# hip-satomi/microbeSEG

Measured on AMD Instinct MI355X. Metric: training crops/sec (256px), higher is better.
Workload: dtype f32; 1 GPU; BASELINE configs[1]: DU-Net distance-map training step, filters [64, 1024], 256x256 crops, per-GPU batch 32, fp32, relu/bn, SmoothL1x2 + Adam(amsgrad); global_batch=32, parallelism=dp1, launch=eager

## Files before the change

### microbeseg_amd/csrc/igemm.hip

```cpp
#include "common.h"
#include "igemm_common.h"
#include "bf16_affine.h"

int igemm_p8_try(const MsegIgemm& p, int tr, int m_fastest, int cus, hipStream_t st);

__device__ float g_ident_scale[MSEG_MAX_CH];
__device__ float g_ident_shift[MSEG_MAX_CH];
__global__ void init_ident_kernel() {
  for (int i = blockIdx.x * blockDim.x + threadIdx.x; i < MSEG_MAX_CH; i += gridDim.x * blockDim.x) {
    g_ident_scale[i] = 1.f;
    g_ident_shift[i] = 0.f;
  }
}


template <int BM, int BN, bool PER_SAMPLE, bool GENERIC_ACT>
__global__ __launch_bounds__(256) void igemm_kernel(const MsegIgemm p) {
  using Cfg = IgemmCfg<BM, BN>;
  constexpr int STAGE = (BM + BN) * LDS_STRIDE;
  __shared__ __attribute__((aligned(16))) float lds[2 * STAGE + 4];
  unsigned* tapmask_s = reinterpret_cast<unsigned*>(lds + 2 * STAGE);

  const int tid = threadIdx.x;
  const int lane = tid & 63;
  const int wave = tid >> 6;
  const int wm = wave / Cfg::WN, wn = wave % Cfg::WN;

  const int M = p.NB * p.Ho * p.Wo;
  const int ntiles_n = (p.Ngemm + BN - 1) / BN;
  const int lid = (int)xcd_logical_id(blockIdx.x, gridDim.x);
  const int tile_m = lid / ntiles_n;
  const int tile_n = lid - tile_m * ntiles_n;
  const int m0 = tile_m * BM, n0 = tile_n * BN;

  const int T = p.KH * p.KW;
  const int srow = tid >> 3;
  const int scol = tid & 7;

  const TapGeom geom = make_geom(p);
  RowInfo rows[Cfg::AROWS];
#pragma unroll
  for (int i = 0; i < Cfg::AROWS; ++i) rows[i] = decode_row(p, m0 + srow + 32 * i, M);

  unsigned tapmask = (T >= 32) ? 0xffffffffu : ((1u << T) - 1u);
  if (p.mode == MSEG_MODE_TCONV && p.stride == 2) {
    if (tid == 0) *tapmask_s = 0u;
    __syncthreads();
    unsigned mine = 0u;
    for (int t = 0; t < T; ++t) {
      const int ky = t / p.KW, kx = t - ky * p.KW;
      bool any = false;
#pragma unroll
      for (int i = 0; i < Cfg::AROWS; ++i) {
        int iy, ix;
        any |= tap_coord(geom, rows[i], ky, kx, iy, ix);
      }
      if (any) mine |= (1u << t);
    }
    if (mine) atomicOr(tapmask_s, mine);
    __syncthreads();
    tapmask = *tapmask_s;
    __syncthreads();
  }

  f32x16 acc[Cfg::MB][Cfg::NB];
#pragma unroll
  for (int a = 0; a < Cfg::MB; ++a)
#pragma unroll
    for (int b = 0; b < Cfg::NB; ++b)
#pragma unroll
      for (int r = 0; r < 16; ++r) acc[a][b][r] = 0.f;

  const int nchunks = (p.Cin + KC - 1) / KC;
  const int C0 = p.src[0].C;

  constexpr int NSC = PER_SAMPLE ? Cfg::AROWS : 1;
  float4 ra[Cfg::AROWS], rb[Cfg::BROWS], rsc[NSC], rsh[NSC];
  unsigned amask = 0u;
  int ract = 0;

  auto issue = [&](int chunk, int t, int ky, int kx) {
    const int c = chunk * KC + scol * 4;
    const bool cvalid = c < p.Cin;
    const bool s1 = (p.nsrc > 1) & (c >= C0);
    const float* sptr = s1 ? p.src[1].ptr : p.src[0].ptr;
    const float* sscale = s1 ? p.src[1].scale : p.src[0].scale;
    const float* sshift = s1 ? p.src[1].shift : p.src[0].shift;
    const unsigned sC = (unsigned)(s1 ? p.src[1].C : p.src[0].C);
    const unsigned sss = (unsigned)(s1 ? p.src[1].ss : p.src[0].ss);
    ract = s1 ? p.src[1].act : p.src[0].act;
    const unsigned cl = cvalid ? (unsigned)(s1 ? c - C0 : c) : 0u;
    amask = 0u;
#pragma unroll
    for (int i = 0; i < Cfg::AROWS; ++i) {
      int iy, ix;
      const bool ok = cvalid & tap_coord(geom, rows[i], ky, kx, iy, ix);
      const unsigned pix = (unsigned)((rows[i].n * p.Hi + iy) * p.Wi + ix) & (0u - (unsigned)ok);
      const size_t off = (size_t)pix * sC + (cl & (0u - (unsigned)ok));
      ra[i] = *reinterpret_cast<const float4*>(sptr + off);
      amask |= (unsigned)ok << i;
    }
    const bool has_aff = sscale != nullptr;
    const float* scp = has_aff ? sscale : g_ident_scale;
    const float* shp = has_aff ? sshift : g_ident_shift;
#pragma unroll
    for (int i = 0; i < NSC; ++i) {
      const unsigned n = PER_SAMPLE ? (unsigned)(rows[i].n < 0 ? 0 : rows[i].n) : 0u;
      const size_t o = (size_t)n * (has_aff ? sss : 0u) + cl;
      rsc[i] = *reinterpret_cast<const float4*>(scp + o);
      rsh[i] = *reinterpret_cast<const float4*>(shp + o);
    }
    const float* wt = p.w + ((size_t)t * p.Npad) * p.Kpad;
#pragma unroll
    for (int i = 0; i < Cfg::BROWS; ++i)
      rb[i] = *reinterpret_cast<const float4*>(wt + (size_t)(n0 + srow + 32 * i) * p.Kpad + c);
  };

  auto commit = [&](float* As, float* Bs) {
    const float lo = (ract == MSEG_ACT_RELU) ? 0.f : -3.402823466e38f;
#pragma unroll
    for (int i = 0; i < Cfg::AROWS; ++i) {
      float4 v = ra[i];
      if (GENERIC_ACT) {
        v = act_fwd4(v, ract);
      } else {
        v.x = fmaxf(v.x, lo); v.y = fmaxf(v.y, lo); v.z = fmaxf(v.z, lo); v.w = fmaxf(v.w, lo);
      }
      const float4 sc = rsc[PER_SAMPLE ? i : 0], sh = rsh[PER_SAMPLE ? i : 0];
      const bool ok = (amask >> i) & 1u;
      v.x = ok ? v.x * sc.x + sh.x : 0.f;
      v.y = ok ? v.y * sc.y + sh.y : 0.f;
      v.z = ok ? v.z * sc.z + sh.z : 0.f;
      v.w = ok ? v.w * sc.w + sh.w : 0.f;
      *reinterpret_cast<float4*>(As + (srow + 32 * i) * LDS_STRIDE + scol * 4) = v;
    }
#pragma unroll
    for (int i = 0; i < Cfg::BROWS; ++i)
      *reinterpret_cast<float4*>(Bs + (srow + 32 * i) * LDS_STRIDE + scol * 4) = rb[i];
  };

  struct Pos { int chunk, t, ky, kx; };
  const int KWm1 = p.KW - 1;
  auto advance = [&](Pos q, bool& ok) -> Pos {
    ok = true;
    for (;;) {
      const int wrap = (q.kx == KWm1) ? 1 : 0;
      q.t += 1;
      q.kx = wrap ? 0 : q.kx + 1;
      q.ky += wrap;
      if (q.t >= T) {
        q.t = 0; q.ky = 0; q.kx = 0; q.chunk += 1;
        if (q.chunk >= nchunks) { ok = false; return q; }
      }
      if (tapmask & (1u << q.t)) return q;
    }
  };

  Pos pos = {0, -1, 0, -1};
  bool have = false;
  if (tapmask != 0u) pos = advance(pos, have);
  int cur = 0;
  if (have) {
    issue(pos.chunk, pos.t, pos.ky, pos.kx);
    commit(lds, lds + BM * LDS_STRIDE);
  }
  __syncthreads();

#ifdef MSEG_ABLATE
  const int abl = p.Cq >> 16;
  if ((abl & 16) && ((blockIdx.x >> 8) & 1)) {
    __builtin_amdgcn_s_sleep(48);
  }
  long long t_issue = 0, t_mfma = 0, t_commit = 0, t_bar = 0;
#define STAMP(var) do { if (abl & 32) { __builtin_amdgcn_sched_barrier(0); var = __builtin_amdgcn_s_memtime(); __builtin_amdgcn_s_waitcnt(0xC07F); __builtin_amdgcn_sched_barrier(0); } } while (0)
  long long s0 = 0, s1 = 0, s2 = 0, s3 = 0, s4 = 0;
#else
#define STAMP(var)
#endif
  const int li = lane & 31, lh = lane >> 5;
  while (have) {
    bool have_next;
    const Pos nxt = advance(pos, have_next);
    if (have_next) pos = nxt;
    STAMP(s0);
#ifdef MSEG_ABLATE
    if (!(abl & 1))
#endif
    issue(pos.chunk, pos.t, pos.ky, pos.kx);
    STAMP(s1);

    const float* As = lds + cur * STAGE;
    const float* Bs = As + BM * LDS_STRIDE;
#pragma unroll
    for (int kk = 0; kk < KC / 8; ++kk) {
      float4 af[Cfg::MB], bf[Cfg::NB];
#pragma unroll
      for (int a = 0; a < Cfg::MB; ++a)
        af[a] = *reinterpret_cast<const float4*>(As + (wm * Cfg::TM + a * 32 + li) * LDS_STRIDE + kk * 8 + lh * 4);
#pragma unroll
      for (int b = 0; b < Cfg::NB; ++b)
        bf[b] = *reinterpret_cast<const float4*>(Bs + (wn * Cfg::TN + b * 32 + li) * LDS_STRIDE + kk * 8 + lh * 4);
#ifdef MSEG_ABLATE
      if (abl & 4) { asm volatile("" :: "v"(af[0].x), "v"(bf[0].x)); continue; }
#endif
#pragma unroll
      for (int a = 0; a < Cfg::MB; ++a)
#pragma unroll
        for (int b = 0; b < Cfg::NB; ++b) {
          acc[a][b] = __builtin_amdgcn_mfma_f32_32x32x2f32(af[a].x, bf[b].x, acc[a][b], 0, 0, 0);
          acc[a][b] = __builtin_amdgcn_mfma_f32_32x32x2f32(af[a].y, bf[b].y, acc[a][b], 0, 0, 0);
          acc[a][b] = __builtin_amdgcn_mfma_f32_32x32x2f32(af[a].z, bf[b].z, acc[a][b], 0, 0, 0);
          acc[a][b] = __builtin_amdgcn_mfma_f32_32x32x2f32(af[a].w, bf[b].w, acc[a][b], 0, 0, 0);
        }
    }
    float* An = lds + (cur ^ 1) * STAGE;
#ifdef MSEG_ABLATE
    STAMP(s2);
    if (!(abl & 8)) commit(An, An + BM * LDS_STRIDE);
    STAMP(s3);
    if (!(abl & 2)) __syncthreads();
    STAMP(s4);
    t_issue += s1 - s0; t_mfma += s2 - s1; t_commit += s3 - s2; t_bar += s4 - s3;
#else
    commit(An, An + BM * LDS_STRIDE);
    __syncthreads();
#endif
    cur ^= 1;
    have = have_next;
  }

#ifdef MSEG_ABLATE
  if ((abl & 32) && p.dst1 && lane == 0 && blockIdx.x < 1024) {
    float* dbg = p.dst1 + ((size_t)blockIdx.x * 4 + wave) * 4;
    dbg[0] = (float)t_issue; dbg[1] = (float)t_mfma; dbg[2] = (float)t_commit; dbg[3] = (float)t_bar;
  }
#endif
  igemm_epilogue<IgemmCfg<BM, BN>>(acc, m0, n0, wm, wn, lane, M);
}

template <int BM, int BN, int TR, bool PER_SAMPLE, bool SB = false>
__global__ __launch_bounds__(256) void igemm_fast_kernel(const MsegIgemm p) {
  using Cfg = IgemmCfg<BM, BN>;
  constexpr int STAGE = (BM + BN) * LDS_STRIDE;
  __shared__ __attribute__((aligned(16))) float lds[(SB ? 1 : 2) * STAGE];

  const int tid = threadIdx.x;
  const int lane = tid & 63;
  const int wave = tid >> 6;
  const int wm = wave / Cfg::WN, wn = wave % Cfg::WN;
  const int M = p.NB * p.Ho * p.Wo;
  const int ntiles_n = (p.Ngemm + BN - 1) / BN;
  const int lid = (int)xcd_logical_id(blockIdx.x, gridDim.x);
  const int tile_m = lid / ntiles_n;
  const int tile_n = lid - tile_m * ntiles_n;
  const int m0 = tile_m * BM, n0 = tile_n * BN;
  const int T = p.KH * p.KW;
  const int srow = tid >> 3, scol = tid & 7;

  const TapGeom geom = make_geom(p);
  const long long tile_px = tile_base_pixel(p, geom, m0, M);
  int pix0[Cfg::AROWS];
  int rown[Cfg::AROWS];
  unsigned vmask[Cfg::AROWS];
#pragma unroll
  for (int i = 0; i < Cfg::AROWS; ++i) {
    const RowInfo r = decode_row(p, m0 + srow + 32 * i, M);
    const int iy0 = (r.oy * geom.sm - geom.dir * geom.pad) >> geom.sh, ix0 = (r.ox * geom.sm - geom.dir * geom.pad) >> geom.sh;
    pix0[i] = (int)(((long long)r.n * p.Hi + iy0) * p.Wi + ix0 - tile_px);
    rown[i] = r.n < 0 ? 0 : r.n;
    unsigned mk = 0u;
    for (int t = 0; t < T; ++t) {
      const int ky = t / p.KW, kx = t - ky * p.KW;
      int iy, ix;
      mk |= (unsigned)tap_coord(geom, r, ky, kx, iy, ix) << t;
    }
    vmask[i] = mk;
  }

  f32x16 acc[Cfg::MB][Cfg::NB];
#pragma unroll
  for (int a = 0; a < Cfg::MB; ++a)
#pragma unroll
    for (int b = 0; b < Cfg::NB; ++b)
#pragma unroll
      for (int r = 0; r < 16; ++r) acc[a][b][r] = 0.f;

  const int nchunks = (p.Cin + KC - 1) / KC;
  const int C0 = p.src[0].C;
  const unsigned OOB = 0x80000000u;

  const __amdgpu_buffer_rsrc_t rs0 = __builtin_amdgcn_make_buffer_rsrc(
      const_cast<float*>(p.src[0].ptr + tile_px * p.src[0].C), 0, 0x7ffffff0, 0x00020000);
  const __amdgpu_buffer_rsrc_t rs1 = __builtin_amdgcn_make_buffer_rsrc(
      const_cast<float*>((p.nsrc > 1 ? p.src[1].ptr : p.src[0].ptr) + tile_px * (p.nsrc > 1 ? p.src[1].C : p.src[0].C)), 0,
      0x7ffffff0, 0x00020000);
  const __amdgpu_buffer_rsrc_t rsw = __builtin_amdgcn_make_buffer_rsrc(const_cast<float*>(p.w), 0,
                                                                        T * p.Npad * p.Kpad * 4, 0x00020000);
  unsigned wvoff[Cfg::BROWS];
#pragma unroll
  for (int i = 0; i < Cfg::BROWS; ++i) wvoff[i] = ((unsigned)(n0 + srow + 32 * i) * (unsigned)p.Kpad + scol * 4u) * 4u;

  constexpr int NSC = (TR == 0) ? 1 : (PER_SAMPLE ? Cfg::AROWS : 1);
  float4 ra[Cfg::AROWS], rb[Cfg::BROWS], rsc[NSC], rsh[NSC];
  float rm[Cfg::AROWS];
  unsigned rowoff[Cfg::AROWS];
  int ract = 0;
  int cur_chunk = -1;
// ... 1994 lines not shown
  }
  auto tap_at = [&](int j) -> unsigned { return (unsigned)((j < 8 ? taplist >> (8 * j) : taplist_hi >> (8 * (j - 8))) & 0xffull); };
  int chunk = 0, j = 0;
  const int nsteps = nchunks * nlive;
  unsigned e0 = tap_at(0);
  issue(0, (int)(e0 & 15u), (int)((e0 >> 4) & 3u), (int)(e0 >> 6));
  commit(lds, lds + BM * HB_STRIDE);
  __syncthreads();
  int cur = 0;
  const int li = lane & 31, lh = lane >> 5;
  for (int step = 0; step < nsteps; ++step) {
    if (step + 1 < nsteps) {
      j += 1;
      if (j >= nlive) { j = 0; ++chunk; }
    }
    e0 = tap_at(j);
    issue(chunk, (int)(e0 & 15u), (int)((e0 >> 4) & 3u), (int)(e0 >> 6));

    const __bf16* As = lds + cur * STAGE;
    const __bf16* Bs = As + BM * HB_STRIDE;
#pragma unroll
    for (int kk = 0; kk < KC / 16; ++kk) {
      bf16x8 af[Cfg::MB], bf[Cfg::NB];
#pragma unroll
      for (int a = 0; a < Cfg::MB; ++a)
        af[a] = *reinterpret_cast<const bf16x8*>(As + (wm * Cfg::TM + a * 32 + li) * HB_STRIDE + kk * 16 + lh * 8);
#pragma unroll
      for (int b = 0; b < Cfg::NB; ++b)
        bf[b] = *reinterpret_cast<const bf16x8*>(Bs + (wn * Cfg::TN + b * 32 + li) * HB_STRIDE + kk * 16 + lh * 8);
#pragma unroll
      for (int a = 0; a < Cfg::MB; ++a)
#pragma unroll
        for (int b = 0; b < Cfg::NB; ++b)
          acc[a][b] = __builtin_amdgcn_mfma_f32_32x32x16_bf16(af[a], bf[b], acc[a][b], 0, 0, 0);
    }
    __bf16* An = lds + (cur ^ 1) * STAGE;
    commit(An, An + BM * HB_STRIDE);
    __syncthreads();
    cur ^= 1;
  }
  igemm_epilogue<IgemmCfg<BM, BN>>(acc, m0, n0, wm, wn, lane, M);
}

__global__ void igemm_splitk_reduce_kernel(const float* __restrict__ ws, int ksplit, size_t M, int N,
                                           const float* __restrict__ bias, float* __restrict__ dst0, int ld0, int acc0,
                                           float* __restrict__ dst1, int ld1, int acc1, int split, int d16) {
  const int N4 = N >> 2;
  const size_t total = M * (size_t)N4;
  for (size_t i = (size_t)blockIdx.x * blockDim.x + threadIdx.x; i < total; i += (size_t)gridDim.x * blockDim.x) {
    const size_t m = i / N4;
    const int n = (int)(i - m * N4) * 4;
    float4 s = *reinterpret_cast<const float4*>(ws + m * N + n);
    for (int k = 1; k < ksplit; ++k) {
      const float4 v = *reinterpret_cast<const float4*>(ws + ((size_t)k * M + m) * N + n);
      s.x += v.x; s.y += v.y; s.z += v.z; s.w += v.w;
    }
    if (bias) { s.x += bias[n]; s.y += bias[n + 1]; s.z += bias[n + 2]; s.w += bias[n + 3]; }
    const bool second = n >= split;
    void* base = second ? (void*)dst1 : (void*)dst0;
    const size_t e = second ? m * ld1 + (n - split) : m * ld0 + n;
    if (second ? acc1 : acc0) {
      const float4 o = ld_f4_rt(base, e, d16);
      s.x += o.x; s.y += o.y; s.z += o.z; s.w += o.w;
    }
    st_f4_rt(base, e, s, d16);
  }
}

static int check_src(const MsegSrc& s) {
  if (!s.ptr || s.C <= 0 || (s.C & 3)) return MSEG_EINVAL;
  if (s.dtype != MSEG_ST_F32 && s.dtype != MSEG_ST_BF16) return MSEG_EINVAL;
  if (s.dtype == MSEG_ST_BF16 && (s.C & 7)) return MSEG_EINVAL;
  if ((s.scale == nullptr) != (s.shift == nullptr)) return MSEG_EINVAL;
  if (s.scale && (s.ss & 3)) return MSEG_EINVAL;
  return MSEG_OK;
}

static int halo_ksplit(long long htiles, int nchunks, int* chunks_per_split) {
  int ks = 1;
  if (htiles < 256 && nchunks >= 4) {
    long long want = (512 + htiles - 1) / htiles;
    ks = (int)(want < 16 ? want : 16);
    if (ks > nchunks / 2) ks = nchunks / 2;
    if (ks < 1) ks = 1;
  }
  *chunks_per_split = (nchunks + ks - 1) / ks;
  return (nchunks + *chunks_per_split - 1) / *chunks_per_split;
}

static int g_c64p_on = 1;
extern "C" int mseg_igemm_set_persistent(int on) {
  g_c64p_on = on ? 1 : 0;
  return MSEG_OK;
}

static int c64p_workgroups() {
  static int cached[64] = {0};
  int dev = 0;
  if (hipGetDevice(&dev) != hipSuccess || dev < 0 || dev >= 64) return 256;
  if (!cached[dev]) {
    int n = 0;
    if (hipDeviceGetAttribute(&n, hipDeviceAttributeMultiprocessorCount, dev) != hipSuccess || n <= 0) n = 256;
    cached[dev] = n;
  }
  return cached[dev];
}

static long long halo_big_tiles(const MsegIgemm& p, int tw_log2, int BMv) {
  const int TH = BMv >> tw_log2;
  const long long rows = (long long)((p.Hi + TH - 1) / TH) * TH;
  if ((long long)p.Hi * 5 < rows * 4) return 0;
  return (long long)p.NB * ((p.Hi + TH - 1) / TH) * (p.Wi >> tw_log2);
}
static long long halo512_tiles(const MsegIgemm& p, int tw_log2) { return halo_big_tiles(p, tw_log2, 512); }

static int g_w4m_on = 1;
extern "C" int mseg_igemm_set_wide_tiles(int on) {
  g_w4m_on = on ? 1 : 0;
  return MSEG_OK;
}

static bool halo_geometry(const MsegIgemm& p, int BNv, int* tw_log2_out, long long* htiles_out) {
  if (!(p.KH == 3 && p.KW == 3 && p.stride == 1 && p.pad == 1 && p.Ho == p.Hi && p.Wo == p.Wi &&
        p.epi == MSEG_EPI_PLAIN && p.morder == MSEG_MORDER_LINEAR && (p.Wi % 4) == 0))
    return false;
  int tw_log2 = p.precision == MSEG_PREC_BF16 ? 5 : 6;
  while ((p.Wi & ((1 << tw_log2) - 1)) != 0) --tw_log2;
  const int TH = 128 >> tw_log2;
  const long long mt = (long long)p.NB * ((p.Hi + TH - 1) / TH) * (p.Wi >> tw_log2);
  *htiles_out = mt * ((p.Ngemm + BNv - 1) / BNv);
  *tw_log2_out = tw_log2;
  if (p.precision == MSEG_PREC_BF16) return (long long)p.Hi * 2 >= (long long)((p.Hi + TH - 1) / TH) * TH;
  return (long long)p.Hi * 5 >= (long long)((p.Hi + TH - 1) / TH) * TH * 4;
}

extern "C" size_t mseg_igemm_workspace_bytes(const MsegIgemm* pp) {
  if (!pp) return 0;
  const MsegIgemm& p = *pp;
  if (p.Ngemm <= 0 || p.Cin <= 0 || p.NB <= 0 || p.Hi <= 0 || p.Wi <= 0) return 0;
  int tw_log2 = 0, cps = 0;
  long long htiles = 0;
  if (!halo_geometry(p, p.Ngemm > 64 ? 128 : 64, &tw_log2, &htiles)) return 0;
  const int ks = halo_ksplit(htiles, (p.Cin + KC - 1) / KC, &cps);
  if (ks <= 1 || (p.Ngemm & 3)) return 0;
  return (size_t)ks * p.NB * p.Hi * p.Wi * p.Ngemm * sizeof(float);
}

static int igemm_dispatch(const MsegIgemm* pp, void* stream) {
  if (!pp) return MSEG_EINVAL;
  const MsegIgemm& p = *pp;
  if (p.nsrc < 1 || p.nsrc > 2) return MSEG_EINVAL;
  int csum = 0;
  for (int i = 0; i < p.nsrc; ++i) {
    if (check_src(p.src[i])) return MSEG_EINVAL;
    csum += p.src[i].C;
  }
  if (csum != p.Cin) return MSEG_EINVAL;
  if (!p.w || !p.dst0 || p.Kpad < p.Cin || (p.Kpad % KC) || p.Npad < p.Ngemm || (p.Npad % 128)) return MSEG_EINVAL;
  if (p.Cin > MSEG_MAX_CH) return MSEG_EINVAL;
  if (p.NB <= 0 || p.Hi <= 0 || p.Wi <= 0 || p.Ho <= 0 || p.Wo <= 0) return MSEG_EINVAL;
  if (p.KH <= 0 || p.KW <= 0 || p.KH * p.KW > 16) return MSEG_EINVAL;
  if (p.stride != 1 && p.stride != 2) return MSEG_EINVAL;
  if (p.mode != MSEG_MODE_CONV && p.mode != MSEG_MODE_TCONV) return MSEG_EINVAL;
  if (p.morder == MSEG_MORDER_PARITY && ((p.Ho | p.Wo) & 1)) return MSEG_EINVAL;
  if (p.Ngemm <= 0) return MSEG_EINVAL;
  if (p.precision != MSEG_PREC_F32 && p.precision != MSEG_PREC_BF16) return MSEG_EINVAL;
  if (p.dst_dtype != MSEG_ST_F32 && p.dst_dtype != MSEG_ST_BF16) return MSEG_EINVAL;
  const bool s16 = p.src[0].dtype == MSEG_ST_BF16;
  if (p.nsrc > 1 && p.src[1].dtype != p.src[0].dtype) return MSEG_EINVAL;
  if ((s16 || p.dst_dtype == MSEG_ST_BF16) && p.precision != MSEG_PREC_BF16) return MSEG_EINVAL;
  if (p.dst_dtype == MSEG_ST_BF16) {
    if ((p.Ngemm | p.ld0 | p.ld1 | p.Cq) & 1) return MSEG_EINVAL;
    if (p.split < p.Ngemm && (p.split & 1)) return MSEG_EINVAL;
    if (((uintptr_t)p.dst0 | (uintptr_t)p.dst1) & 3) return MSEG_EINVAL;
  }
  if (p.epi == MSEG_EPI_SCATTER2X2) {
    if (p.Cq <= 0 || p.Ngemm != 4 * p.Cq || p.morder != MSEG_MORDER_LINEAR) return MSEG_EINVAL;
  } else if (p.epi == MSEG_EPI_PLAIN) {
    if (p.split < p.Ngemm && !p.dst1) return MSEG_EINVAL;
  } else {
    return MSEG_EINVAL;
  }
  const long long M = (long long)p.NB * p.Ho * p.Wo;
  if (M <= 0 || M > 0x7fffffffLL) return MSEG_EINVAL;
  hipStream_t st = (hipStream_t)stream;
  mseg_dispatch_note(p.precision, 0);
  static bool ident_ready[64] = {false};
  int devid = 0;
  const bool dry = mseg_dispatch_dry() != 0;
  if (!dry) {
    if (hipGetDevice(&devid) != hipSuccess || devid < 0 || devid >= 64) return MSEG_ELAUNCH;
    if (!ident_ready[devid]) {
      MSEG_KL_AUX(init_ident_kernel, dim3(8), dim3(256), 0, st);
      MSEG_LAUNCH_CHECK();
      ident_ready[devid] = true;
    }
  }
  bool per_sample = false, generic = false;
  for (int i = 0; i < p.nsrc; ++i) {
    if (p.src[i].scale && p.src[i].ss != 0) per_sample = true;
    if (p.src[i].act != MSEG_ACT_NONE && p.src[i].act != MSEG_ACT_RELU) generic = true;
  }
  const bool wide = p.Ngemm > 64;
  const int BMv = 128, BNv = wide ? 128 : 64;
  const long long tiles = ((M + BMv - 1) / BMv) * ((p.Ngemm + BNv - 1) / BNv);
  if (tiles > 0x7fffffffLL) return MSEG_EINVAL;
  const dim3 grid((unsigned)tiles), block(256);
  bool fast = (p.mode == MSEG_MODE_CONV) || (p.stride == 1) ||
              (p.morder == MSEG_MORDER_PARITY && (M % (4 * BMv)) == 0);
  bool plain = true, band_fits = true;
  for (int i = 0; i < p.nsrc; ++i) {
    if (((128LL / p.Wo + 3) * p.stride + p.KH) * p.Wi * p.src[i].C * 4 >= 0x7ffffff0LL) fast = false;
    if (34LL * p.Wi * p.src[i].C * 4 >= 0x80000000LL) band_fits = false;
    if (p.src[i].act != MSEG_ACT_NONE || p.src[i].scale) plain = false;
  }
  bool common = true;
  if ((long long)p.KH * p.KW * p.Npad * p.Kpad * 4 >= 0x80000000LL) common = false;
  if (p.KH > 4 || p.KW > 4) common = false;
  if (p.nsrc > 1 && (p.src[0].C % KC)) common = false;
  fast = fast && common;
  int tw_log2 = 6;
  long long htiles = 0;
  if (common && band_fits && halo_geometry(p, BNv, &tw_log2, &htiles) && htiles <= 0x7fffffffLL) {
    const int tr = plain ? 0 : (generic ? 2 : 1);
    int cps = 0;
    int ks = halo_ksplit(htiles, (p.Cin + KC - 1) / KC, &cps);
    const size_t need = (size_t)ks * (size_t)M * (size_t)p.Ngemm * sizeof(float);
    if (ks > 1 && (!p.ws || p.ws_bytes < need || (p.Ngemm & 3) || (p.split & 3) || htiles * ks > 0x7fffffffLL)) {
      ks = 1;
      cps = (p.Cin + KC - 1) / KC;
    }
    MsegIgemm q = p;
    if (ks > 1) {
      q.dst0 = (float*)p.ws; q.dst1 = nullptr; q.ld0 = p.Ngemm; q.ld1 = 0; q.split = p.Ngemm; q.acc0 = 0; q.acc1 = 0;
      q.bias = nullptr;
      q.dst_dtype = MSEG_ST_F32;
    }
    mseg_dispatch_note(p.precision, ks > 1 ? need : 0);
    const dim3 hgrid((unsigned)(htiles * ks));
#define MSEG_HALO(BN_, TR_) MSEG_KL((igemm_halo_kernel<BN_, TR_>), hgrid, dim3(512), 0, st, q, tw_log2, ks, cps)
    const int m_fastest = ((long long)9 * p.Kpad * p.Ngemm * 2 > (2ll << 20)) && (p.Ngemm > BNv) ? 1 : 0;
#define MSEG_HALO16(BN_, TR_)                                                                                          \
  do {                                                                                                                 \
    if (s16) MSEG_KL((igemm_halo_bf16_kernel<BN_, TR_, true>), hgrid, dim3(512), 0, st, q, tw_log2, ks, cps, m_fastest); \
    else MSEG_KL((igemm_halo_bf16_kernel<BN_, TR_, false>), hgrid, dim3(512), 0, st, q, tw_log2, ks, cps, m_fastest);    \
  } while (0)
#define MSEG_HALO16W4(TR_)                                                                                             \
  do {                                                                                                                 \
    if (s16) MSEG_KL((igemm_halo_bf16w4_kernel<TR_, true>), hgrid, dim3(256), 0, st, q, tw_log2, ks, cps, m_fastest);    \
    else MSEG_KL((igemm_halo_bf16w4_kernel<TR_, false>), hgrid, dim3(256), 0, st, q, tw_log2, ks, cps, m_fastest);       \
  } while (0)
    int p8rc = 0;
    if (p.precision == MSEG_PREC_BF16 && s16 && !wide && g_c64p_on && p.nsrc == 1 && p.Cin == 64 && p.Kpad == 64 &&
        ks == 1 && tw_log2 <= 5 && p.split >= p.Ngemm && htiles >= 4 * (long long)c64p_workgroups()) {
      const int wgs = c64p_workgroups();
      const dim3 pgrid((unsigned)wgs);
#define MSEG_C64P(TR_)                                                                                                        \
  do {                                                                                                                         \
    if (q.dst_dtype == MSEG_ST_BF16) MSEG_KL((igemm_c64p_bf16_kernel<TR_, true>), pgrid, dim3(512), 0, st, q, tw_log2, (int)htiles); \
    else MSEG_KL((igemm_c64p_bf16_kernel<TR_, false>), pgrid, dim3(512), 0, st, q, tw_log2, (int)htiles);               \
  } while (0)
      if (tr == 0) MSEG_C64P(0); else if (tr == 1) MSEG_C64P(1); else MSEG_C64P(2);
#undef MSEG_C64P
    } else if (p.precision == MSEG_PREC_BF16 && !wide && g_c64p_on && p.Cin >= 128 && ks == 1 && tw_log2 >= 4 &&
               halo512_tiles(p, tw_log2) >= 2 * (long long)c64p_workgroups()) {
      const dim3 mgrid((unsigned)halo512_tiles(p, tw_log2));
#define MSEG_HALO512(TR_)                                                                                                      \
  do {                                                                                                                         \
    if (s16) MSEG_KL((igemm_halo_bf16m512_kernel<TR_, true>), mgrid, dim3(512), 0, st, q, tw_log2, 1, cps, 0);      \
    else MSEG_KL((igemm_halo_bf16m512_kernel<TR_, false>), mgrid, dim3(512), 0, st, q, tw_log2, 1, cps, 0);         \
  } while (0)
      if (tr == 0) MSEG_HALO512(0); else if (tr == 1) MSEG_HALO512(1); else MSEG_HALO512(2);
#undef MSEG_HALO512
    } else if (p.precision == MSEG_PREC_BF16 && wide && s16 && ks == 1 &&
               (p8rc = igemm_p8_try(q, tr, m_fastest, c64p_workgroups(), st)) != 0) {
      if (p8rc < 0) return p8rc;
    } else if (p.precision == MSEG_PREC_BF16 && wide && s16 && g_w4m_on && ks == 1 && tw_log2 >= 3 &&
               halo_big_tiles(p, tw_log2, 256) * ((p.Ngemm + 127) / 128) >= 2 * (long long)c64p_workgroups()) {
      const dim3 mgrid((unsigned)(halo_big_tiles(p, tw_log2, 256) * ((p.Ngemm + 127) / 128)));
#define MSEG_HALOW4M(TR_) \
  MSEG_KL((igemm_halo_bf16w4m_kernel<TR_, true>), mgrid, dim3(256), 0, st, q, tw_log2, 1, cps, m_fastest)
      if (tr == 0) MSEG_HALOW4M(0); else if (tr == 1) MSEG_HALOW4M(1); else MSEG_HALOW4M(2);
#undef MSEG_HALOW4M
    } else if (p.precision == MSEG_PREC_BF16) {
      if (wide) { if (tr == 0) MSEG_HALO16W4(0); else if (tr == 1) MSEG_HALO16W4(1); else MSEG_HALO16W4(2); }
      else      { if (tr == 0) MSEG_HALO16(64, 0); else if (tr == 1) MSEG_HALO16(64, 1); else MSEG_HALO16(64, 2); }
    } else if (wide) { if (tr == 0) MSEG_HALO(128, 0); else if (tr == 1) MSEG_HALO(128, 1); else MSEG_HALO(128, 2); }
    else      { if (tr == 0) MSEG_HALO(64, 0); else if (tr == 1) MSEG_HALO(64, 1); else MSEG_HALO(64, 2); }
#undef MSEG_HALO
#undef MSEG_HALO16
#undef MSEG_HALO16W4
    MSEG_LAUNCH_CHECK();
    if (ks > 1) {
      const size_t total = (size_t)M * (size_t)(p.Ngemm >> 2);
      size_t blocks = (total + 255) / 256;
      if (blocks > 16384) blocks = 16384;
      MSEG_KL_AUX(igemm_splitk_reduce_kernel, dim3((unsigned)blocks), dim3(256), 0, st, (const float*)p.ws, ks,
                         (size_t)M, p.Ngemm, p.bias, p.dst0, p.ld0, p.acc0, p.dst1, p.ld1, p.acc1,
                         p.split < p.Ngemm ? p.split : p.Ngemm, p.dst_dtype == MSEG_ST_BF16 ? 1 : 0);
      MSEG_LAUNCH_CHECK();
    }
    return MSEG_OK;
  }
  if (p.precision == MSEG_PREC_BF16 && s16 && g_c64p_on && p.epi == MSEG_EPI_SCATTER2X2 && p.KH == 1 && p.KW == 1 &&
      p.stride == 1 && p.pad == 0 && p.mode == MSEG_MODE_CONV && p.nsrc == 1 && p.Cin == 128 && p.Kpad == 128 &&
      p.Cq == 64 && p.Ngemm == 256 && !p.acc0 && (p.Wi % 32) == 0 && (((long long)p.Hi * p.Wi) % 128) == 0 &&
      M / 128 >= 4 * (long long)c64p_workgroups()) {
    const int tr = plain ? 0 : (generic ? 2 : 1);
    const dim3 pgrid((unsigned)c64p_workgroups());
    const int nt = (int)(M / 128);
#define MSEG_CTP(TR_)                                                                                                \
  do {                                                                                                               \
    if (p.dst_dtype == MSEG_ST_BF16) MSEG_KL((igemm_ctp_bf16_kernel<TR_, true>), pgrid, dim3(512), 0, st, p, nt); \
    else MSEG_KL((igemm_ctp_bf16_kernel<TR_, false>), pgrid, dim3(512), 0, st, p, nt);                     \
  } while (0)
    if (tr == 0) MSEG_CTP(0); else if (tr == 1) MSEG_CTP(1); else MSEG_CTP(2);
#undef MSEG_CTP
    MSEG_LAUNCH_CHECK();
    return MSEG_OK;
  }
  if (p.precision == MSEG_PREC_BF16 && s16 && g_c64p_on && p.epi == MSEG_EPI_SCATTER2X2 && p.KH == 1 && p.KW == 1 &&
      p.stride == 1 && p.pad == 0 && p.mode == MSEG_MODE_CONV && p.nsrc == 1 && p.Cin == 256 && p.Kpad == 256 &&
      p.Cq == 128 && p.Ngemm == 512 && !p.acc0 && p.Wi >= 32 && (((long long)p.Hi * p.Wi) % 64) == 0 &&
      (c64p_workgroups() & 3) == 0 && M / 64 >= 4 * (long long)(c64p_workgroups() / 4)) {
    const int tr = plain ? 0 : (generic ? 2 : 1);
    const dim3 pgrid((unsigned)c64p_workgroups());
    const int nt = (int)(M / 64);
#define MSEG_CTP2(TR_)                                                                                               \
  do {                                                                                                               \
    if (p.dst_dtype == MSEG_ST_BF16) MSEG_KL((igemm_ctp2_bf16_kernel<TR_, true>), pgrid, dim3(512), 0, st, p, nt); \
    else MSEG_KL((igemm_ctp2_bf16_kernel<TR_, false>), pgrid, dim3(512), 0, st, p, nt);                    \
  } while (0)
    if (tr == 0) MSEG_CTP2(0); else if (tr == 1) MSEG_CTP2(1); else MSEG_CTP2(2);
#undef MSEG_CTP2
    MSEG_LAUNCH_CHECK();
    return MSEG_OK;
  }
  if (p.precision == MSEG_PREC_BF16 && s16 && g_c64p_on && plain && p.epi == MSEG_EPI_PLAIN && p.KH == 2 && p.KW == 2 &&
      p.stride == 2 && p.pad == 0 && p.mode == MSEG_MODE_CONV && p.morder == MSEG_MORDER_LINEAR && p.nsrc == 1 &&
      p.Cin == 64 && p.Kpad == 64 && p.Ngemm == 128 && p.split >= p.Ngemm && !p.acc0 && !p.bias && (p.Wo % 32) == 0 &&
      p.Hi == 2 * p.Ho && p.Wi == 2 * p.Wo && (M % 64) == 0 && M / 64 >= 4 * (long long)c64p_workgroups()) {
    const dim3 pgrid((unsigned)c64p_workgroups());
    if (p.dst_dtype == MSEG_ST_BF16) MSEG_KL((igemm_ctd_bf16_kernel<true>), pgrid, dim3(512), 0, st, p, (int)(M / 64));
    else MSEG_KL((igemm_ctd_bf16_kernel<false>), pgrid, dim3(512), 0, st, p, (int)(M / 64));
    MSEG_LAUNCH_CHECK();
    return MSEG_OK;
  }
  if (p.precision == MSEG_PREC_BF16) {
    if (!fast) return MSEG_EINVAL;
    const int tr = plain ? 0 : (generic ? 2 : 1);
#define MSEG_FAST16_LAUNCH(BM_, BN_, TR_, PS_)                                                          \
  do {                                                                                                  \
    if (s16) MSEG_KL((igemm_fast_bf16_kernel<BM_, BN_, TR_, PS_, true>), grid, block, 0, st, p);   \
    else MSEG_KL((igemm_fast_bf16_kernel<BM_, BN_, TR_, PS_, false>), grid, block, 0, st, p);      \
  } while (0)
#define MSEG_FAST16_TILE(BM_, BN_)                                                        \
  do {                                                                                    \
    if (tr == 0) MSEG_FAST16_LAUNCH(BM_, BN_, 0, false);                                  \
    else if (tr == 1) { if (per_sample) MSEG_FAST16_LAUNCH(BM_, BN_, 1, true); else MSEG_FAST16_LAUNCH(BM_, BN_, 1, false); } \
    else { if (per_sample) MSEG_FAST16_LAUNCH(BM_, BN_, 2, true); else MSEG_FAST16_LAUNCH(BM_, BN_, 2, false); }              \
  } while (0)
    if (wide) MSEG_FAST16_TILE(128, 128); else MSEG_FAST16_TILE(128, 64);
#undef MSEG_FAST16_TILE
#undef MSEG_FAST16_LAUNCH
    MSEG_LAUNCH_CHECK();
    return MSEG_OK;
  }
  if (fast) {
    const int tr = plain ? 0 : (generic ? 2 : 1);
    const int live_taps = (p.mode == MSEG_MODE_TCONV && p.stride == 2) ? ((p.KH + 1) / 2) * ((p.KW + 1) / 2) : p.KH * p.KW;
    const bool short_k = ((p.Cin + KC - 1) / KC) * live_taps <= 8;
#define MSEG_FAST_LAUNCH(BM_, BN_, TR_, PS_)                                                              \
  do {                                                                                                    \
    if (short_k) MSEG_KL((igemm_fast_kernel<BM_, BN_, TR_, PS_, true>), grid, block, 0, st, p); \
    else MSEG_KL((igemm_fast_kernel<BM_, BN_, TR_, PS_, false>), grid, block, 0, st, p);        \
  } while (0)
#define MSEG_FAST_TILE(BM_, BN_)                                                          \
  do {                                                                                    \
    if (tr == 0) MSEG_FAST_LAUNCH(BM_, BN_, 0, false);                                    \
    else if (tr == 1) { if (per_sample) MSEG_FAST_LAUNCH(BM_, BN_, 1, true); else MSEG_FAST_LAUNCH(BM_, BN_, 1, false); } \
    else { if (per_sample) MSEG_FAST_LAUNCH(BM_, BN_, 2, true); else MSEG_FAST_LAUNCH(BM_, BN_, 2, false); }              \
  } while (0)
    if (wide) MSEG_FAST_TILE(128, 128); else MSEG_FAST_TILE(128, 64);
#undef MSEG_FAST_TILE
#undef MSEG_FAST_LAUNCH
    MSEG_LAUNCH_CHECK();
    return MSEG_OK;
  }
#define MSEG_IGEMM_LAUNCH(BM_, BN_, PS_, GA_) \
  MSEG_KL((igemm_kernel<BM_, BN_, PS_, GA_>), grid, block, 0, st, p)
  if (wide) {
    if (per_sample) { if (generic) MSEG_IGEMM_LAUNCH(128, 128, true, true); else MSEG_IGEMM_LAUNCH(128, 128, true, false); }
    else            { if (generic) MSEG_IGEMM_LAUNCH(128, 128, false, true); else MSEG_IGEMM_LAUNCH(128, 128, false, false); }
  } else {
    if (per_sample) { if (generic) MSEG_IGEMM_LAUNCH(128, 64, true, true); else MSEG_IGEMM_LAUNCH(128, 64, true, false); }
    else            { if (generic) MSEG_IGEMM_LAUNCH(128, 64, false, true); else MSEG_IGEMM_LAUNCH(128, 64, false, false); }
  }
#undef MSEG_IGEMM_LAUNCH
  MSEG_LAUNCH_CHECK();
  return MSEG_OK;
}

extern "C" int mseg_igemm(const MsegIgemm* pp, void* stream) {
  mseg_dispatch_begin(0);
  const int rc = igemm_dispatch(pp, stream);
  mseg_dispatch_end(nullptr);
  return rc;
}

extern "C" int mseg_igemm_query(const MsegIgemm* pp, MsegKernelInfo* info) {
  if (!info) return MSEG_EINVAL;
  mseg_dispatch_begin(1);
  const int rc = igemm_dispatch(pp, nullptr);
  mseg_dispatch_end(info);
  return rc;
}

__global__ void f32_to_bf16_kernel(const float* __restrict__ src, __bf16* __restrict__ dst, size_t n) {
  for (size_t i = (size_t)blockIdx.x * blockDim.x + threadIdx.x; i < n; i += (size_t)gridDim.x * blockDim.x)
    dst[i] = (__bf16)src[i];
}

extern "C" int mseg_f32_to_bf16(const float* src, uint16_t* dst, size_t n, void* stream) {
  if (!src || !dst || n == 0) return MSEG_EINVAL;
  size_t blocks = (n + 255) / 256;
  if (blocks > 8192) blocks = 8192;
  hipLaunchKernelGGL(f32_to_bf16_kernel, dim3((unsigned)blocks), dim3(256), 0, (hipStream_t)stream, src, (__bf16*)dst, n);
  MSEG_LAUNCH_CHECK();
  return MSEG_OK;
}

__global__ void pack_weight_kernel(const float* __restrict__ src, float* __restrict__ dst, int T, int R, int Rpad,
                                   int C, int Cpad, int st, int sr, int sc) {
  const size_t total = (size_t)T * Rpad * Cpad;
  for (size_t i = (size_t)blockIdx.x * blockDim.x + threadIdx.x; i < total; i += (size_t)gridDim.x * blockDim.x) {
    const int c = (int)(i % Cpad);
    const size_t tr = i / Cpad;
    const int r = (int)(tr % Rpad);
    const int t = (int)(tr / Rpad);
    dst[i] = (c < C && r < R) ? src[(size_t)t * st + (size_t)r * sr + (size_t)c * sc] : 0.f;
  }
}

extern "C" int mseg_pack_weight(const float* src, float* dst, int T, int R, int Rpad, int C, int Cpad, int st, int sr,
                                int sc, void* stream) {
  if (!src || !dst || T <= 0 || R <= 0 || Rpad < R || C <= 0 || Cpad < C || (Cpad & 3)) return MSEG_EINVAL;
  const size_t total = (size_t)T * Rpad * Cpad;
  unsigned blocks = (unsigned)((total + 255) / 256);
  if (blocks > 4096u) blocks = 4096u;
  hipLaunchKernelGGL(pack_weight_kernel, dim3(blocks), dim3(256), 0, (hipStream_t)stream, src, dst, T, R, Rpad, C,
                     Cpad, st, sr, sc);
  MSEG_LAUNCH_CHECK();
  return MSEG_OK;
}

#define PACK_TILE 32
__global__ __launch_bounds__(256) void pack_weights_multi_kernel(const MsegPackJob* __restrict__ jobs, int njobs) {
  __shared__ float tile[PACK_TILE * (PACK_TILE * 9 + 1)];
  int lo = 0, hi = njobs - 1;
  const unsigned b = blockIdx.x;
  while (lo < hi) {
    const int mid = (lo + hi + 1) >> 1;
    if (jobs[mid].first_block <= b) lo = mid; else hi = mid - 1;
  }
  const MsegPackJob j = jobs[lo];
  const int T = j.T;
  const int ctiles = (j.Cpad + PACK_TILE - 1) / PACK_TILE;
  const int tb = (int)(b - j.first_block);
  const int r0 = (tb / ctiles) * PACK_TILE, c0 = (tb % ctiles) * PACK_TILE;
  const bool inner_c = j.sc <= j.sr;
  const int run = PACK_TILE * T, pitch = run + 1;
  const int o0 = inner_c ? r0 : c0, i0 = inner_c ? c0 : r0;
  const int on = inner_c ? j.R : j.C, in = inner_c ? j.C : j.R;
  const long long so = inner_c ? j.sr : j.sc, si = inner_c ? j.sc : j.sr;
  const bool contiguous = j.st == 1 && si == T;
  for (int e = threadIdx.x; e < PACK_TILE * run; e += 256) {
    const int o = e / run, k = e - o * run;
    const int i = k / T, t = k - i * T;
    float v = 0.f;
    if (o0 + o < on && i0 + i < in)
      v = contiguous ? j.src[(long long)(o0 + o) * so + (long long)i0 * T + k]
                     : j.src[(long long)t * j.st + (long long)(o0 + o) * so + (long long)(i0 + i) * si];
    tile[o * pitch + k] = v;
  }
  __syncthreads();
  const int c = threadIdx.x & 31;
  for (int q = threadIdx.x >> 5; q < PACK_TILE * T; q += 8) {
    const int r = q % PACK_TILE, t = q / PACK_TILE;
    if (r0 + r >= j.Rpad || c0 + c >= j.Cpad) continue;
    const float v = inner_c ? tile[r * pitch + c * T + t] : tile[c * pitch + r * T + t];
    const size_t d = ((size_t)t * j.Rpad + r0 + r) * j.Cpad + c0 + c;
    if (j.dst) j.dst[d] = v;
    if (j.dst16) ((__bf16*)j.dst16)[d] = (__bf16)v;
  }
}

extern "C" unsigned mseg_pack_job_blocks(int T, int Rpad, int Cpad) {
  if (T <= 0 || T > 9 || Rpad <= 0 || Cpad <= 0) return 0;
  return (unsigned)(((Rpad + PACK_TILE - 1) / PACK_TILE) * ((Cpad + PACK_TILE - 1) / PACK_TILE));
}

extern "C" int mseg_pack_weights_multi(const MsegPackJob* jobs_dev, int njobs, unsigned total_blocks, void* stream) {
  if (!jobs_dev || njobs <= 0 || total_blocks == 0) return MSEG_EINVAL;
  hipLaunchKernelGGL(pack_weights_multi_kernel, dim3(total_blocks), dim3(256), 0, (hipStream_t)stream, jobs_dev, njobs);
  MSEG_LAUNCH_CHECK();
  return MSEG_OK;
}
```

Measured before the change: 242.7 crops/s.

## Add persistent fp32 MFMA implicit-GEMM kernel for transposed-conv and 2x2 stride-2 convs

Adds a new persistent-grid fp32 implicit-GEMM kernel (128x128 tiles, 512 threads, double-buffered LDS, 32x32x2 f32 MFMA) for two shapes: the 1x1 scatter-2x2 transposed-conv forward and the 2x2 stride-2 pooling-style conv. Each workgroup loops over tiles, prefetching the next tile's first chunk while it finishes the current one, and writes results through a buffer-resource epilogue that handles the scatter layout directly. The kernel is tried before the existing dispatch paths whenever the fp32 shape conditions hold. It adds a new code path with its own offset-overflow guards, and the fixed tile shape and occupancy may be a worse fit than the existing kernels for some layer sizes.

```diff
diff --git a/microbeseg_amd/csrc/igemm.hip b/microbeseg_amd/csrc/igemm.hip
--- a/microbeseg_amd/csrc/igemm.hip
+++ b/microbeseg_amd/csrc/igemm.hip
@@ -3,6 +3,7 @@
 #include "bf16_affine.h"
 
 int igemm_p8_try(const MsegIgemm& p, int tr, int m_fastest, int cus, hipStream_t st);
+int igemm_ct_try(const MsegIgemm& p, int tr, hipStream_t st);
 
 __device__ float g_ident_scale[MSEG_MAX_CH];
 __device__ float g_ident_shift[MSEG_MAX_CH];
@@ -2603,6 +2604,11 @@
     }
     return MSEG_OK;
   }
+  {
+    const int ctrc = igemm_ct_try(p, plain ? 0 : (generic ? 2 : 1), st);
+    if (ctrc < 0) return ctrc;
+    if (ctrc > 0) return MSEG_OK;
+  }
   if (p.precision == MSEG_PREC_BF16 && s16 && g_c64p_on && p.epi == MSEG_EPI_SCATTER2X2 && p.KH == 1 && p.KW == 1 &&
       p.stride == 1 && p.pad == 0 && p.mode == MSEG_MODE_CONV && p.nsrc == 1 && p.Cin == 128 && p.Kpad == 128 &&
       p.Cq == 64 && p.Ngemm == 256 && !p.acc0 && (p.Wi % 32) == 0 && (((long long)p.Hi * p.Wi) % 128) == 0 &&
diff --git a/microbeseg_amd/csrc/igemm_ct.hip b/microbeseg_amd/csrc/igemm_ct.hip
--- /dev/null
+++ b/microbeseg_amd/csrc/igemm_ct.hip
@@ -0,0 +1,249 @@
+#include "common.h"
+#include "igemm_common.h"
+
+int igemm_ct_try(const MsegIgemm& p, int tr, hipStream_t st);
+
+template <int BN>
+struct CtCfg {
+  static constexpr int WN = 4, WM = 2;
+  static constexpr int TM = 128 / WM, TN = BN / WN;
+  static constexpr int MB = TM / 32, NB = TN / 32;
+};
+
+template <typename Cfg, bool SCATTER, typename AccT>
+__device__ __forceinline__ void ct_epilogue_regular(AccT& acc, int m0, int n0, int wm, int wn, int lane) {
+  const int li = lane & 31, lh = lane >> 5;
+  const MsegIgemm* pe = (const MsegIgemm*)__builtin_amdgcn_kernarg_segment_ptr();
+  asm volatile("" : "+s"(pe));
+  const float* e_bias = pe->bias;
+  float* e_dst0 = pe->dst0;
+  const int e_ld0 = pe->ld0, e_acc0 = pe->acc0, e_Cq = pe->Cq, e_Ho = pe->Ho, e_Wo = pe->Wo, e_Ngemm = pe->Ngemm;
+#pragma unroll
+  for (int b = 0; b < Cfg::NB; ++b) {
+    const int nb0 = n0 + wn * Cfg::TN + b * 32;
+    if (nb0 >= e_Ngemm) continue;
+    const bool nvalid = nb0 + li < e_Ngemm;
+    const int ab = SCATTER ? nb0 / e_Cq : 0;
+    const int col0 = SCATTER ? nb0 - ab * e_Cq : nb0;
+    const int sa = ab >> 1, sb = ab & 1;
+    const int step = SCATTER ? 2 * e_Cq : e_ld0;
+    const float bias = (e_bias && nvalid) ? e_bias[col0 + li] : 0.f;
+    const unsigned vo = nvalid ? (unsigned)(li + 4 * lh * step) * 4u : 0x80000000u;
+#pragma unroll
+    for (int a = 0; a < Cfg::MB; ++a) {
+      const int mb = m0 + wm * Cfg::TM + a * 32;
+      size_t tb;
+      if (SCATTER) {
+        const int img = mb / (e_Ho * e_Wo);
+        const int rem = mb - img * (e_Ho * e_Wo);
+        const int y = rem / e_Wo, x = rem - y * e_Wo;
+        tb = (((size_t)img * (2 * e_Ho) + 2 * y + sa) * (2 * e_Wo) + 2 * x + sb) * e_Cq + col0;
+      } else {
+        tb = (size_t)mb * e_ld0 + col0;
+      }
+      const __amdgpu_buffer_rsrc_t rd = __builtin_amdgcn_make_buffer_rsrc(e_dst0 + tb, 0, 0x7ffffff0, 0x00020000);
+      float old[16];
+#pragma unroll
+      for (int r = 0; r < 16; ++r) old[r] = 0.f;
+      if (e_acc0) {
+#pragma unroll
+        for (int r = 0; r < 16; ++r)
+          old[r] = __builtin_bit_cast(float, __builtin_amdgcn_raw_buffer_load_b32(rd, vo, ((r & 3) + 8 * (r >> 2)) * step * 4, 0));
+      }
+#pragma unroll
+      for (int r = 0; r < 16; ++r) {
+        const float v = acc[a][b][r] + bias + old[r];
+        __builtin_amdgcn_raw_buffer_store_b32(__builtin_bit_cast(unsigned, v), rd, vo, ((r & 3) + 8 * (r >> 2)) * step * 4, 0);
+      }
+    }
+  }
+}
+
+template <int BN, int TR, bool DG>
+__global__ __launch_bounds__(512, 4) void igemm_ct_kernel(const MsegIgemm p, int ntiles) {
+  constexpr int BM = 128;
+  using Cfg = CtCfg<BN>;
+  constexpr int STAGE = (BM + BN) * LDS_STRIDE;
+  constexpr int AR = BM / 64, BR = BN / 64;
+  constexpr int T = DG ? 4 : 1;
+  __shared__ __attribute__((aligned(16))) float lds[2 * STAGE];
+
+  const int tid = threadIdx.x, lane = tid & 63, wave = tid >> 6;
+  const int wm = wave / Cfg::WN, wn = wave % Cfg::WN;
+  const int li = lane & 31, lh = lane >> 5;
+  const int srow = tid >> 3, scol = tid & 7;
+  const int M = p.NB * p.Ho * p.Wo;
+  const int ntiles_n = (p.Ngemm + BN - 1) / BN;
+  const int C = p.Cin;
+  const int nsteps = (C / KC) * T;
+  const unsigned C4 = (unsigned)C * 4u;
+  const unsigned OOB = 0x80000000u;
+  const int G = (int)gridDim.x;
+  const int wm_s = __builtin_amdgcn_readfirstlane(wm), wn_s = __builtin_amdgcn_readfirstlane(wn);
+  const bool regular_shape = DG || (p.Wo & 31) == 0;
+
+  const __amdgpu_buffer_rsrc_t rsw = __builtin_amdgcn_make_buffer_rsrc(const_cast<float*>(p.w), 0,
+                                                                        T * p.Npad * p.Kpad * 4, 0x00020000);
+  __amdgpu_buffer_rsrc_t rsa;
+  unsigned rowoff[AR], wvoff[BR];
+  int l_m0 = 0, l_n0 = 0;
+  auto setup = [&](int tile) {
+    const int tile_m = tile / ntiles_n;
+    l_m0 = tile_m * BM;
+    l_n0 = (tile - tile_m * ntiles_n) * BN;
+    const int q0 = DG ? l_m0 / p.Wo : 0;
+    const long long px0 = DG ? 2ll * l_m0 + 2ll * p.Wo * q0 : (long long)l_m0;
+    rsa = __builtin_amdgcn_make_buffer_rsrc(const_cast<float*>(p.src[0].ptr + px0 * C), 0, 0x7ffffff0, 0x00020000);
+#pragma unroll
+    for (int i = 0; i < AR; ++i) {
+      const int r = srow + 64 * i, m = l_m0 + r;
+      const unsigned rel = DG ? (unsigned)(2 * r + 2 * p.Wo * (m / p.Wo - q0)) : (unsigned)r;
+      rowoff[i] = m < M ? rel * C4 + scol * 16u : OOB;
+    }
+#pragma unroll
+    for (int i = 0; i < BR; ++i) wvoff[i] = ((unsigned)(l_n0 + srow + 64 * i) * (unsigned)p.Kpad + scol * 4u) * 4u;
+  };
+
+  float4 ra[AR], rb[BR];
+  float4 rsc = make_float4(1.f, 1.f, 1.f, 1.f), rsh = make_float4(0.f, 0.f, 0.f, 0.f);
+  const float lo = (TR != 0 && p.src[0].act == MSEG_ACT_RELU) ? 0.f : -3.402823466e38f;
+
+  auto issue = [&](int chunk, int t) {
+    const unsigned aso = (unsigned)chunk * (KC * 4u) + (DG ? (unsigned)((t >> 1) * p.Wi + (t & 1)) * C4 : 0u);
+#pragma unroll
+    for (int i = 0; i < AR; ++i) {
+      const f32x4 v = __builtin_bit_cast(f32x4, __builtin_amdgcn_raw_buffer_load_b128(rsa, rowoff[i], aso, 0));
+      ra[i] = make_float4(v[0], v[1], v[2], v[3]);
+    }
+    if (TR != 0 && p.src[0].scale != nullptr && (!DG || t == 0)) {
+      rsc = *reinterpret_cast<const float4*>(p.src[0].scale + chunk * KC + scol * 4);
+      rsh = *reinterpret_cast<const float4*>(p.src[0].shift + chunk * KC + scol * 4);
+    }
+    const unsigned wso = ((unsigned)t * (unsigned)p.Npad * (unsigned)p.Kpad + (unsigned)chunk * KC) * 4u;
+#pragma unroll
+    for (int i = 0; i < BR; ++i) {
+      const f32x4 v = __builtin_bit_cast(f32x4, __builtin_amdgcn_raw_buffer_load_b128(rsw, wvoff[i], wso, 0));
+      rb[i] = make_float4(v[0], v[1], v[2], v[3]);
+    }
+  };
+
+  auto commit = [&](float* As, float* Bs) {
+#pragma unroll
+    for (int i = 0; i < AR; ++i) {
+      float4 v = ra[i];
+      if (TR != 0) {
+        v.x = clamp_lo(v.x, lo); v.y = clamp_lo(v.y, lo); v.z = clamp_lo(v.z, lo); v.w = clamp_lo(v.w, lo);
+        v.x = v.x * rsc.x + rsh.x; v.y = v.y * rsc.y + rsh.y; v.z = v.z * rsc.z + rsh.z; v.w = v.w * rsc.w + rsh.w;
+      }
+      *reinterpret_cast<float4*>(As + (srow + 64 * i) * LDS_STRIDE + scol * 4) = v;
+    }
+#pragma unroll
+    for (int i = 0; i < BR; ++i)
+      *reinterpret_cast<float4*>(Bs + (srow + 64 * i) * LDS_STRIDE + scol * 4) = rb[i];
+  };
+
+  int tile = __builtin_amdgcn_readfirstlane((int)xcd_logical_id(blockIdx.x, gridDim.x));
+  if (tile >= ntiles) return;
+  setup(tile);
+  int lc = 0, lt = 0;
+  issue(0, 0);
+  commit(lds, lds + BM * LDS_STRIDE);
+  __syncthreads();
+  int cur = 0;
+  for (;;) {
+    const int c_m0 = l_m0, c_n0 = l_n0;
+    const int next_tile = tile + G;
+    f32x16 acc[Cfg::MB][Cfg::NB];
+#pragma unroll
+    for (int a = 0; a < Cfg::MB; ++a)
+#pragma unroll
+      for (int b = 0; b < Cfg::NB; ++b)
+#pragma unroll
+        for (int r = 0; r < 16; ++r) acc[a][b][r] = 0.f;
+
+    for (int step = 0; step < nsteps; ++step) {
+      if (step + 1 < nsteps) {
+        if (++lt == T) { lt = 0; ++lc; }
+      } else if (next_tile < ntiles) {
+        setup(next_tile);
+        lc = 0; lt = 0;
+      }
+      issue(lc, lt);
+
+      const float* As = lds + cur * STAGE;
+      const float* Bs = As + BM * LDS_STRIDE;
+#pragma unroll
+      for (int kk = 0; kk < KC / 8; ++kk) {
+        float4 af[Cfg::MB], bf[Cfg::NB];
+#pragma unroll
+        for (int a = 0; a < Cfg::MB; ++a)
+          af[a] = *reinterpret_cast<const float4*>(As + (wm * Cfg::TM + a * 32 + li) * LDS_STRIDE + kk * 8 + lh * 4);
+#pragma unroll
+        for (int b = 0; b < Cfg::NB; ++b)
+          bf[b] = *reinterpret_cast<const float4*>(Bs + (wn * Cfg::TN + b * 32 + li) * LDS_STRIDE + kk * 8 + lh * 4);
+#pragma unroll
+        for (int a = 0; a < Cfg::MB; ++a)
+#pragma unroll
+          for (int b = 0; b < Cfg::NB; ++b) {
+            acc[a][b] = __builtin_amdgcn_mfma_f32_32x32x2f32(af[a].x, bf[b].x, acc[a][b], 0, 0, 0);
+            acc[a][b] = __builtin_amdgcn_mfma_f32_32x32x2f32(af[a].y, bf[b].y, acc[a][b], 0, 0, 0);
+            acc[a][b] = __builtin_amdgcn_mfma_f32_32x32x2f32(af[a].z, bf[b].z, acc[a][b], 0, 0, 0);
+            acc[a][b] = __builtin_amdgcn_mfma_f32_32x32x2f32(af[a].w, bf[b].w, acc[a][b], 0, 0, 0);
+          }
+      }
+      float* An = lds + (cur ^ 1) * STAGE;
+      commit(An, An + BM * LDS_STRIDE);
+      __syncthreads();
+      cur ^= 1;
+    }
+    if (regular_shape && c_m0 + BM <= M) ct_epilogue_regular<Cfg, !DG>(acc, c_m0, c_n0, wm_s, wn_s, lane);
+    else igemm_epilogue<Cfg>(acc, c_m0, c_n0, wm, wn, lane, M);
+    if (next_tile >= ntiles) break;
+    tile = next_tile;
+  }
+}
+
+static int ct_compute_units() {
+  static int cached[64] = {0};
+  int dev = 0;
+  if (hipGetDevice(&dev) != hipSuccess || dev < 0 || dev >= 64) return 256;
+  if (!cached[dev]) {
+    int n = 0;
+    if (hipDeviceGetAttribute(&n, hipDeviceAttributeMultiprocessorCount, dev) != hipSuccess || n <= 0) n = 256;
+    cached[dev] = n;
+  }
+  return cached[dev];
+}
+
+int igemm_ct_try(const MsegIgemm& p, int tr, hipStream_t st) {
+  if (p.precision != MSEG_PREC_F32 || p.dst_dtype != MSEG_ST_F32 || p.nsrc != 1 || p.src[0].dtype != MSEG_ST_F32) return 0;
+  const MsegSrc& s = p.src[0];
+  if (tr != 0 && tr != 1) return 0;
+  if (s.scale && s.ss != 0) return 0;
+  if (s.C < KC || (s.C % KC) || p.Cin != s.C) return 0;
+  if (p.mode != MSEG_MODE_CONV || p.morder != MSEG_MORDER_LINEAR || p.pad != 0) return 0;
+  const bool fwd = p.KH == 1 && p.KW == 1 && p.stride == 1 && p.epi == MSEG_EPI_SCATTER2X2 && p.Hi == p.Ho &&
+                   p.Wi == p.Wo && p.Cq >= KC && (p.Cq % KC) == 0;
+  const bool dg = p.KH == 2 && p.KW == 2 && p.stride == 2 && p.epi == MSEG_EPI_PLAIN && p.Hi == 2 * p.Ho &&
+                  p.Wi == 2 * p.Wo && p.split >= p.Ngemm;
+  if (!fwd && !dg) return 0;
+  if ((long long)(fwd ? 2 * (long long)p.Cq : (long long)p.ld0) * 32 * 4 >= 0x7ffffff0LL || (dg && p.ld0 < p.Ngemm)) return 0;
+  if ((long long)p.KH * p.KW * p.Npad * p.Kpad * 4 >= 0x80000000LL) return 0;
+  if (dg && (2LL * 127 + 2LL * p.Wo * (127 / p.Wo + 1) + p.Wi + 2) * s.C * 4 >= 0x7ffffff0LL) return 0;
+  const long long M = (long long)p.NB * p.Ho * p.Wo;
+  const long long tiles = ((M + 127) / 128) * ((p.Ngemm + 127) / 128);
+  const int cus = ct_compute_units();
+  if (tiles < cus || tiles > 0x3fffffffLL) return 0;
+  const long long slots = 2LL * cus;
+  const dim3 grid((unsigned)(tiles < slots ? tiles : slots)), block(512);
+  const int nt = (int)tiles;
+  if (dg) {
+    if (tr == 0) MSEG_KL((igemm_ct_kernel<128, 0, true>), grid, block, 0, st, p, nt);
+    else MSEG_KL((igemm_ct_kernel<128, 1, true>), grid, block, 0, st, p, nt);
+  } else {
+    if (tr == 0) MSEG_KL((igemm_ct_kernel<128, 0, false>), grid, block, 0, st, p, nt);
+    else MSEG_KL((igemm_ct_kernel<128, 1, false>), grid, block, 0, st, p, nt);
+  }
+  MSEG_LAUNCH_CHECK();
+  return 1;
+}
```

Result: no change. 244.6 crops/s (median of 6 runs) (+0.8%).
